# OrangeSodahub/InfGen

Hardware: AMD Instinct MI355X
Metric: agent-steps/sec (closed-loop rollout) (higher is better)
Workload: dtype f32

## Files before the change

### include/infgen_hip.h

```cpp
#ifndef INFGEN_HIP_H_
#define INFGEN_HIP_H_

#include <stdint.h>

#ifdef __cplusplus
extern "C" {
#endif

#define INFGEN_MAX_LAYERS 8

enum {
  INFGEN_Q_ATTN_PACK_SIZE = 0,
  INFGEN_Q_FOURIER_PACK_SIZE_N2 = 1,
  INFGEN_Q_FOURIER_PACK_SIZE_N3 = 2,
  INFGEN_Q_FOURIER_PACK_SIZE_N4 = 3,
  INFGEN_Q_TILE_ROWS = 4,
  INFGEN_Q_EDGE_ATTN_CAP = 5,
  INFGEN_Q_MAX_AGENTS = 6,
  INFGEN_Q_ABI_VERSION = 7,
  INFGEN_Q_SIZEOF_ROLLOUT = 8,
  INFGEN_Q_ATTN_SPLIT_ROWS = 9,
  INFGEN_Q_HEADS_SAMPLE_K = 10,
};
int infgen_layout_query(int what);
// ... 132 lines not shown
int infgen_heads(const float* X, int rows, const float* tok_pack, const float* st_pack, int token_size,
                 float* logits, int* next_token, int* next_state, void* stream);
int infgen_heads_logprob(const float* X, int rows, const float* tok_pack, const float* st_pack, int token_size,
                         float* logits, int* next_token, int* next_state, float* token_logprob, void* stream);
int infgen_token_logprob(const float* logits, int rows, int n, const int* token, float* out, void* stream);
int infgen_heads_sample(const float* X, int rows, const float* tok_pack, const float* st_pack, int token_size, int k,
                        const float* uniform, float* logits, int* next_token, int* next_state, float* token_logprob,
                        float* sample_logprob, void* stream);
int infgen_heads_sample_ex(const float* X, int rows, const float* tok_pack, const float* st_pack, int token_size, int k,
                           const float* uniform, const InfgenSampling* sampling, float* logits, int* next_token, int* next_state,
                           float* token_logprob, float* sample_logprob, void* stream);
int infgen_heads_sample_mask(const float* X, int rows, const float* tok_pack, const float* st_pack, int token_size, int k,
                             const float* uniform, const InfgenSampling* sampling, const uint32_t* mask_bits, int mask_n_sets,
                             const int* mask_row, const int* mask_type, const int* type, float* logits,
                             int* next_token, int* next_state, float* token_logprob, float* sample_logprob, void* stream);
int infgen_heads_sample_fused(int attn_mode, int rows, int k);
int infgen_heads_logprob_fused(int attn_mode, int rows);
int infgen_map_token_head(const float* X, int ldx, const int* gather, int n, const float* pack, int token_size,
                          float* hidden, float* logits, long long* top_idx, void* stream);
int infgen_embedding_sum4(const float* tab0, const long long* idx0, int n0, const float* tab1, const long long* idx1, int n1,
                          const float* tab2, const long long* idx2, int n2, const float* tab3, const long long* idx3, int n3,
                          int rows, float* out, void* stream);
int infgen_map_graph(int S, int M_cap, const int* n_map, const float* pos, const float* orient, float radius,
                     int max_nbr, int* off, int* cnt, int* src, float* raw, int* total, int cap, void* stream);

int infgen_rollout_validate(const InfgenRollout* r);
int infgen_build_edges(const InfgenRollout* r, int c, int edgeless, void* stream);
int infgen_integrate(const InfgenRollout* r, int t, void* stream);
int infgen_raw_feature(const InfgenRollout* r, int col, void* stream);
int infgen_raw_feature_rows(const InfgenRollout* r, int col, const int* row_list, const int* row_mask, int n, void* stream);
int infgen_decode_layers(const InfgenRollout* r, int c, int edgeless, void* stream);
int infgen_decode_step(const InfgenRollout* r, int t, void* stream);
int infgen_rollout_run(const InfgenRollout* r, int t0, int t1, void* stream);
int infgen_command_rows(const InfgenRollout* r, int t, int kind, const int* cmd_token, const float* cmd_pose,
                        const unsigned char* cmd_mask, const float* shape, float* cmd_cost, void* stream);

int infgen_branch_scenes(const InfgenRollout* r, int t, const int* parent, int* n_bad, void* stream);
int infgen_resample_parents(const int* ancestor, int S0, int copies, int* parent, void* stream);

int infgen_snapshot_bytes(const InfgenRollout* r, int t, long long* bytes);
int infgen_snapshot_scenes(const InfgenRollout* r, int t, const int* slots, int n, void* snap, long long entry_stride, int* head,
                           int* n_bad, void* stream);
int infgen_restore_scenes(const InfgenRollout* r, int t, const int* index, const void* snap, long long entry_stride, const int* head,
                          int n, int* n_bad, void* stream);

int infgen_sample_topk(const float* logits, int rows, int n, int k, const float* uniform, int* token, void* stream);
int infgen_sample_topk_logprob(const float* logits, int rows, int n, int k, const float* uniform, int* token,
                               float* sample_logprob, void* stream);
int infgen_sample_topk_ex(const float* logits, int rows, int n, int k, const float* uniform, const InfgenSampling* sampling,
                          int* token, float* sample_logprob, int* nucleus, void* stream);
int infgen_sample_topk_mask(const float* logits, int rows, int n, int k, const float* uniform, const InfgenSampling* sampling,
                            const uint32_t* mask_bits, int mask_n_sets, const int* mask_row, const int* mask_type, const int* type,
                            int* token, float* sample_logprob, int* nucleus, void* stream);
int infgen_token_mask_create(const uint32_t* mask_bits, int mask_n_sets, const int* mask_row, const int* mask_type, const int* type);
int infgen_token_mask_destroy(int handle);

int infgen_collision_end_poses(const float* vocab, int token_size, float* end_pose, void* stream);
int infgen_collision_mask(const float* pos, const float* head, const int* state, const int* n_agents, const int* first_new,
                          const int* type, const float* shape, int S, int A_cap, int T, int c, const float* end_pose, int token_size,
                          int predict, float margin, const uint32_t* mask_bits, int mask_n_sets, const int* mask_row,
                          const int* mask_type, uint32_t* out_bits, int* out_count, void* stream);
int infgen_token_mask_collision(int handle, uint32_t* dyn_bits, const int* identity_row, const float* shape, const float* end_pose,
                                int predict, float margin, int* count);

int infgen_road_records_from_map(const float* map_pos, const float* map_orient, const long long* map_type, const long long* map_tok,
                                 const int* n_map, int S0, int M_cap, const float* map_vocab, int n_token, int detail, float* records,
// ... 221 lines not shown
```

### infgen_amd/csrc/api.hip

```cpp
#include <cstdio>
#include <cstring>
#include <cstdlib>
#include <cmath>
#include <string>
#include <vector>
#include <atomic>
#include <mutex>
#include <unordered_map>
#include "kernels.h"
#include "../../include/infgen_hip.h"

using namespace ig;

static thread_local std::string g_err;

static int fail(const char* where, const char* what) {
  g_err = std::string(where) + ": " + what;
  return -1;
}
static int check_launch(const char* where) {
  hipError_t e = hipGetLastError();
  if (e != hipSuccess) return fail(where, hipGetErrorString(e));
  return 0;
}
// ... 81 lines not shown
static int env_layers_p() { const int v = env_int("INFGEN_LAYERS_P", 1); return v < 0 ? 0 : v > 2 ? 2 : v; }
static int env_lp_rows_min() {
  bool set8 = false;
  const int rows8 = env_int("INFGEN_LP_ROWS8", 0, &set8);
  return set8 ? (rows8 ? 8 : 16) : env_int("INFGEN_LP_ROWS_MIN", 4);
}
namespace knob {
const int layers_p = env_layers_p();
const int qs_dbg = env_int("INFGEN_QS_DBG", 0);
const int fh12_min = env_int("INFGEN_FH12_MIN", 150000);
const int fh12_multi_rows = env_int("INFGEN_FH12_MULTI_ROWS", 0);
const int fourier_nomulti = env_int("INFGEN_FOURIER_NOMULTI", 0);
const int attn_hs_max = env_int("INFGEN_ATTN_HS_MAX", 6144);
const int attn_waves = env_int("INFGEN_ATTN_WAVES", IG_QSU ? 8 : 4);
const int warm = env_int("INFGEN_WARM", 1);
const int warm_max_groups = env_int("INFGEN_WARM_MAX_GROUPS", 128);
const int edge_dbg = env_int("INFGEN_EDGE_DBG", 0);
const int edge_noxcd = env_int("INFGEN_EDGE_NOXCD", 0);
const int edge_small = env_int("INFGEN_EDGE_SMALL", 4096);
const int edge_wg2 = env_int("INFGEN_EDGE_WG2", 1);
const int edge_lds_pad = env_int("INFGEN_EDGE_LDS_PAD", 0);
const int heads_nosplit = env_int("INFGEN_HEADS_NOSPLIT", 0);
const int be_wide_scenes = env_int("INFGEN_BE_WIDE_SCENES", 128);
const int int_group_scenes = env_int("INFGEN_INT_GROUP_SCENES", 128);
const int no_tail_fold = env_int("INFGEN_NO_TAIL_FOLD", 0);
const int lp_max_chunks = env_int("INFGEN_LP_MAX_CHUNKS", 2);
const int lp_max_groups = env_int("INFGEN_LP_MAX_GROUPS", 256);
const int lp_rows_min = env_lp_rows_min();
const int cm_rows = env_int("INFGEN_CM_ROWS", 0);
const int lp_trace = env_int("INFGEN_LP_TRACE", 0);
const char* const lp_spin_str = getenv("INFGEN_LP_SPIN_LIMIT");
const unsigned lp_spin_limit = lp_spin_str ? (unsigned)strtoul(lp_spin_str, nullptr, 0) : 0u;
}

namespace {
InfgenOptions g_def = {0,  2,  3,  1,  1,  6,  0,
                        0,  knob::layers_p,  0,  1, 0, nullptr, nullptr};
int g_def_group_rows = 0;
const int* g_def_limit_n_agents = nullptr;
int g_def_limit_A_cap = 0;
struct Active { const InfgenOptions* o; int group_rows; const int* n_agents; int A_cap; };
thread_local Active tl_active = {nullptr, 0, nullptr, 0};
thread_local InfgenOptions tl_thread_opts;
thread_local bool tl_thread_set = false;
inline const InfgenOptions& O() { return tl_active.o ? *tl_active.o : tl_thread_set ? tl_thread_opts : g_def; }
inline int group_rows() { return tl_active.o ? tl_active.group_rows : g_def_group_rows; }
inline const int* limit_n_agents() { return tl_active.o ? tl_active.n_agents : g_def_limit_n_agents; }
inline int limit_A_cap() { return tl_active.o ? tl_active.A_cap : g_def_limit_A_cap; }
struct OptScope {
  Active prev;
  explicit OptScope(const InfgenRollout* r) : prev(tl_active) {
    if (r && r->opts.use) tl_active = Active{&r->opts, r->S * r->A_cap, r->opts.row_groups ? r->n_agents : nullptr, r->A_cap};
  }
  ~OptScope() { tl_active = prev; }
};
}

extern "C" int infgen_get_options(InfgenOptions* out) {
  if (!out) return fail("infgen_get_options", "null pointer");
  *out = g_def;
  return 0;
}

extern "C" int infgen_thread_options(const InfgenOptions* o) {
  if (o) { tl_thread_opts = *o; tl_thread_opts.row_groups = nullptr; tl_thread_opts.n_row_groups = nullptr; }
  tl_thread_set = o != nullptr;
  return 0;
}

extern "C" int infgen_get_effective_options(InfgenOptions* out) {
  if (!out) return fail("infgen_get_effective_options", "null pointer");
  *out = O();
  return 0;
}

namespace {
struct Prof {
  unsigned mask = 0;
  std::vector<hipEvent_t> e0, e1;
  std::vector<int> kid;
  std::vector<int> phase_of;
  std::vector<double> macs;
  int stride = 1;
  int seen[INFGEN_KID_COUNT] = {};
  int seen_step[INFGEN_KID_COUNT] = {};
  size_t used = 0;
  unsigned long long* rows_dev = nullptr;
} g_prof;

static thread_local int t_prof_phase = 0;
static std::mutex g_prof_mu;
struct ProfScope {
  int slot = -1;
  hipStream_t s;
  ProfScope(int kid, void* stream, double macs = 0.0) : s((hipStream_t)stream) {
    if ((g_prof.mask >> kid) & 1u) {
      std::lock_guard<std::mutex> lk(g_prof_mu);
      ++g_prof.seen[kid];
      const bool take = t_prof_phase != 1 || (g_prof.seen_step[kid]++ % g_prof.stride) == 0;
      if (take && g_prof.used < g_prof.e0.size()) {
        slot = (int)g_prof.used++;
        g_prof.kid[slot] = kid;
        g_prof.phase_of[slot] = t_prof_phase;
        g_prof.macs[slot] = macs;
        (void)hipEventRecord(g_prof.e0[slot], s);
      }
    }
// ... 201 lines not shown
extern "C" int infgen_set_gemm_terms(int terms) {
  if (terms < 1 || terms > 3) return fail("infgen_set_gemm_terms", "terms must be 3 (split, fp32 accuracy), 2 (bf16 operands) or 1 (fp16 operands)");
  g_def.gemm_terms = terms;
  return 0;
}

extern "C" int infgen_set_fourier_mode(int mode) {
  if (mode != 0 && mode != 1) return fail("infgen_set_fourier_mode", "mode must be 0 (fp32 MFMA) or 1 (fp16 split)");
  g_def.fourier_mode = mode;
  return 0;
}

static FourierArgs fourier_args(const float* raw, int n, const int* count_dev, int e_cap, const float* pack, const float* cat, int ldcat,
                                float* out, int ldo, int normalize, int out_r24, const float* dt_tab = nullptr, int dt_mode = 0) {
  return FourierArgs{raw, n, count_dev, e_cap, pack, cat, ldcat, out, ldo, normalize,
                     (g_prof.mask >> INFGEN_KID_FOURIER) & 1u && dt_mode != 2 ? g_prof.rows_dev : nullptr, out_r24, dt_tab, dt_mode, 0};
}

static inline int fourier_h_grid(int cap, bool wide) {
  const int grid = ceil_div(cap, wide ? FH12_TILE : FH_TILE);
  return grid > 256 * FH_WG_PER_CU ? 256 * FH_WG_PER_CU : grid;
}

static int launch_fourier(const FourierArgs& a_in, void* stream) {
  if (a_in.e_cap <= 0) return 0;
  FourierArgs a = a_in;
  a.dbg = knob::qs_dbg;
  { ProfScope _ps(INFGEN_KID_FOURIER, stream);
    if (O().fourier_mode == 0) {
      int grid = ceil_div(a.e_cap, TR);
      if (grid > 2048) grid = 2048;
      hipLaunchKernelGGL(k_fourier, dim3(grid), dim3(NT), 0, (hipStream_t)stream, a);
    } else {
      const bool wide = knob::fh12_min > 0 && a.e_cap >= knob::fh12_min && three_terms() && FH_WAVES == 8;
      const int grid = fourier_h_grid(a.e_cap, wide);
      if (wide) hipLaunchKernelGGL(k_fourier_h12<3>, dim3(grid), dim3(FH12_NT), 0, (hipStream_t)stream, a);
      else hipLaunchKernelGGL(by_terms(k_fourier_h<3>, k_fourier_h_b16<1>, k_fourier_h<1>), dim3(grid), dim3(FH_NT), 0, (hipStream_t)stream, a);
    } }
  return check_launch("infgen_fourier_embed");
}

static int fourier_embed_impl(const float* raw, int n, const int* count_dev, int e_cap, const float* pack,
                              const float* cat, int ldcat, float* out, int ldo, int normalize, int out_r24, void* stream,
                              const float* dt_tab = nullptr, int dt_mode = 0) {
  if (e_cap <= 0) return 0;
  if (n < 1 || n > 4) return fail("infgen_fourier_embed", "n_dims must be in 1..4");
  if (out_r24 && O().fourier_mode == 0) return fail("infgen_fourier_embed", "packed rows need the split kernel");
  if (dt_mode && (O().fourier_mode == 0 || n < 2 || (dt_mode == 1 && !dt_tab)))
    return fail("infgen_fourier_embed", "the last-dim table needs the split kernel, n_dims >= 2 and a table");
  return launch_fourier(fourier_args(raw, n, count_dev, e_cap, pack, cat, ldcat, out, ldo, normalize, out_r24, dt_tab, dt_mode), stream);
}

extern "C" int infgen_fourier_embed(const float* raw, int n, const int* count_dev, int e_cap, const float* pack,
                                    const float* cat, int ldcat, float* out, int ldo, int normalize, void* stream) {
  return fourier_embed_impl(raw, n, count_dev, e_cap, pack, cat, ldcat, out, ldo, normalize, 0, stream);
}

extern "C" int infgen_fourier_last_dim_table(const float* pack, int n, float* table, void* stream) {
  return fourier_embed_impl(nullptr, n, nullptr, DT_TAB_ROWS, pack, nullptr, 0, table, 128, 0, 0, stream, nullptr, 2);
}
extern "C" int infgen_fourier_embed_tab(const float* raw, int n, const int* count_dev, int e_cap, const float* pack,
                                        const float* table, float* out, int ldo, int normalize, void* stream) {
  return fourier_embed_impl(raw, n, count_dev, e_cap, pack, nullptr, 0, out, ldo, normalize, 0, stream, table, 1);
}

extern "C" int infgen_set_attn_mode(int mode) {
  if (mode < 0 || mode > 3) return fail("infgen_set_attn_mode", "mode must be 0 (fp32 MFMA), 1 (fp16 split), 2 (by size) or 3 (fp16 split, 16-row workgroups)");
// ... 1133 lines not shown
    if (coll.bits && (r->token_size % 32 || r->token_size > 64 * 32 * RIDER_WPL))
      return fail(where, "collision mask: token_size must be a multiple of 32, at most 4096");
    if (road.bits && (r->token_size % 32 || r->token_size > 64 * 32 * RIDER_WPL))
      return fail(where, "road mask: token_size must be a multiple of 32, at most 4096");
    if (road.bits && r->S % road.copies) return fail(where, "road mask: S must be a multiple of copies");
    if (score.out && r->first_new)
      return fail(where, "step score: contexts with scenario insertion cannot be scored: rows appended inside a step are left out");
    if (score.out && r->S % score.copies) return fail(where, "step score: S must be a multiple of copies");
  }
  if (r->token_logprob && !(r->store_logits && r->logits) && !r->logits_scratch) {
    const int mode = (r->opts.use ? r->opts : O()).attn_mode;
    const int k = r->sample_k > 1 && r->sample_u ? r->sample_k : 1;
    if (emit_plan(mode, r->S * r->A_cap, r->token_size, k, true, false).need_logits)
      return fail(where, "token_logprob needs store_logits or logits_scratch [rows][token_size] (few rows, or sampling)");
  }
  return 0;
}

static int build_edges_impl(const InfgenRollout* r, int c, int edgeless, void* stream, bool zero_totals, unsigned long long* clear_keys = nullptr,
                            bool clear_sync = false) {
  RET_IF(validate(r, "infgen_build_edges"));
  OptScope _opts(r);
  hipStream_t s = (hipStream_t)stream;
  if (!edgeless && zero_totals) {
    if (r->em.total == r->et.total + 1 && r->ea.total == r->et.total + 2) {
      if (hipMemsetAsync(r->et.total, 0, 3 * sizeof(int), s) != hipSuccess) return fail("infgen_build_edges", "memset failed");
    } else if (hipMemsetAsync(r->et.total, 0, sizeof(int), s) != hipSuccess ||
               hipMemsetAsync(r->em.total, 0, sizeof(int), s) != hipSuccess ||
               hipMemsetAsync(r->ea.total, 0, sizeof(int), s) != hipSuccess)
      return fail("infgen_build_edges", "memset failed");
  }
  BuildEdgesArgs a;
  a.st = scene_of(r); a.c = c; a.edgeless = edgeless; a.r_map = r->r_map; a.r_agent = r->r_agent;
  a.rows = r->S * r->A_cap; a.t = ebuf(r->et); a.m = ebuf(r->em); a.a = ebuf(r->ea);
  a.clear_keys = clear_keys;
  a.clear_sync = clear_sync ? reinterpret_cast<int*>(r->SIG) : nullptr;
  a.prof = (g_prof.mask & ((1u << INFGEN_KID_EDGE_ATTN) | (1u << INFGEN_KID_BUILD_EDGES))) ? g_prof.rows_dev : nullptr;
  { ProfScope _ps(INFGEN_KID_BUILD_EDGES, stream);
    a.map_lds = r->M_cap < 4096 ? r->M_cap : 4096;
    const size_t lds = (size_t)a.map_lds * 8;
    if (r->A_cap <= 256 && r->S > knob::be_wide_scenes) hipLaunchKernelGGL(k_build_edges<256>, dim3(r->S, 3), dim3(256), lds, s, a);
    else hipLaunchKernelGGL(k_build_edges<1024>, dim3(r->S, 3), dim3(1024), lds, s, a); }
  return check_launch("infgen_build_edges");
}
extern "C" int infgen_build_edges(const InfgenRollout* r, int c, int edgeless, void* stream) {
  return build_edges_impl(r, c, edgeless, stream, true);
}

static RawFeatArgs rawfeat_args(const InfgenRollout* r, int col) {
  RawFeatArgs a;
  a.st = scene_of(r); a.col = col; a.tok_tab = r->tok_tab; a.token_size = r->token_size;
  a.grid_tab = r->grid_tab; a.grid_size = r->grid_size; a.state_emb = r->state_emb;
  a.cat_agent = r->cat_agent; a.cat_seed = r->cat_seed; a.raw2 = r->raw2; a.cat = r->cat; a.fus_in = r->fus_in;
  a.row_list = nullptr; a.row_mask = nullptr; a.n_list = 0; a.no_grid = r->no_grid_token;
  return a;
}

static int integrate_groups(const InfgenRollout* r) {
  return (r->S <= knob::int_group_scenes && r->A_cap % 16 == 0 && r->A_cap > 16) ? r->A_cap / 16 : 1;
}
static int integrate_impl(const InfgenRollout* r, int t, void* stream, unsigned long long* heads_part, bool zero_totals, bool prep, bool zero_sync = false) {
  RET_IF(validate(r, "infgen_integrate"));
  OptScope _opts(r);
  IntegrateArgs a;
  a.heads_part = heads_part; a.next_token_w = r->next_token;
  a.edge_totals = zero_totals ? r->et.total : nullptr;
  a.zero_sync = zero_sync ? reinterpret_cast<int*>(r->SIG) : nullptr;
// ... 293 lines not shown
}
extern "C" int infgen_layers_p_capacity(void) {
  const LpDevice& d = lp_device();
  if (d.wg_per_cu <= 0) return 0;
  return d.n_cu * (d.wg_per_cu > 1 ? 1 : d.wg_per_cu);
}
static int lp_limit() {
  const int cap = infgen_layers_p_capacity(), mx = knob::lp_max_groups;
  return cap < mx ? cap : mx;
}
static bool is_capturing(void* stream) {
  hipStreamCaptureStatus cap = hipStreamCaptureStatusNone;
  return hipStreamIsCapturing((hipStream_t)stream, &cap) == hipSuccess && cap != hipStreamCaptureStatusNone;
}
static bool lp_packs_ok(const InfgenRollout* r, bool refresh = false, void* stream = nullptr) {
  static std::mutex mu;
  static std::unordered_map<const float*, bool> seen;
  std::lock_guard<std::mutex> lk(mu);
  const bool capturing = stream && is_capturing(stream);
  auto ok = [&](const float* pack) {
    if (!pack) return false;
    if (!refresh) { auto it = seen.find(pack); if (it != seen.end()) return it->second; }
    if (capturing) return false;
    float hdr[16] = {};
    const bool good = hipMemcpy(hdr, pack + AH_HDR, sizeof(hdr), hipMemcpyDeviceToHost) == hipSuccess && hdr[14] == AH_HDR_VERSION &&
                      hdr[10] > 0.f && hdr[12] > 0.f;
    seen[pack] = good;
    return good;
  };
  for (int i = 0; i < r->num_layers; ++i)
    if (!ok(r->attn_t[i]) || !ok(r->attn_m[i]) || !ok(r->attn_a[i])) return false;
  return true;
}
extern "C" int infgen_rollout_validate(const InfgenRollout* r) {
  RET_IF(validate(r, "infgen_rollout_validate"));
  if (r->replay_row && !(r->teacher_token && r->teacher_state))
    return fail("infgen_rollout_validate", "replay_row needs teacher_token and teacher_state (the plan the flagged rows follow)");
  if ((r->teacher_pos != nullptr) != (r->teacher_head != nullptr))
    return fail("infgen_rollout_validate", "teacher_pos and teacher_head come together");
  (void)lp_packs_ok(r, true);
  return 0;
}
static bool layers_p_shape(const InfgenRollout* r, int rows, int edgeless, void* stream) {
  const LpDevice& lpd = lp_device();
  if (lpd.wg_per_cu <= 0 || (O().layers_p == 2 && (!lpd.coop || g_lp_refused.load()))) return false;
  return O().layers_p && O().edge_fuse != 0 && O().attn_mode != 0 && three_terms() && O().fourier_mode != 0 &&
         !(O().overlap && g_side) && r->A_cap % 16 == 0 && lp_chunk_scenes(r, lp_limit()) > 0 &&
          r->num_layers <= LP_MAX_LAYERS && r->U && r->SIG && !r->tap_x && lp_packs_ok(r, false, stream);
}

struct StepMode { bool overlap, fuse, lp; int r24; int ra; const float* dt; };
static StepMode step_mode(const InfgenRollout* r, int rows, int edgeless, void* stream) {
  StepMode m;
  m.overlap = O().overlap && g_side && !edgeless;
  m.lp = layers_p_shape(r, rows, edgeless, stream);
  m.fuse = O().edge_fuse == 2 || (O().edge_fuse == 1 && (rows > 256 || m.lp));
  m.r24 = m.fuse && O().fourier_mode != 0 && O().rhat_format == 1;
  m.ra = m.r24;
  m.dt = O().fourier_mode != 0 ? r->four_t_dt : nullptr;
  return m;
}
static bool fourier_multi_ok(int rows, int edgeless) {
  return !edgeless && O().fourier_mode != 0 && rows <= 10240 && !knob::fourier_nomulti && !(O().overlap && g_side);
}

enum FourierSet { FS_TEMPORAL, FS_MAP, FS_AGENT, FS_XA };
static FourierArgs step_fourier_set(const InfgenRollout* r, FourierSet k, const StepMode& sm) {
  switch (k) {
    case FS_TEMPORAL:
      return fourier_args(r->et.raw, 4, r->et.total, r->et.cap, r->four_t, nullptr, 0, r->et.rhat, 128, 1, sm.r24, sm.dt, sm.dt != nullptr);
    case FS_MAP: return fourier_args(r->em.raw, 3, r->em.total, r->em.cap, r->four_m, nullptr, 0, r->em.rhat, 128, 1, sm.r24);
    case FS_AGENT: return fourier_args(r->ea.raw, 3, r->ea.total, r->ea.cap, r->four_a, nullptr, 0, r->ea.rhat, 128, 1, sm.ra);
    default: return fourier_args(r->raw2, 2, nullptr, r->S * r->A_cap, r->four_xa, r->cat, 128, r->fus_in + 128, 512, 0, 0);
// ... 13 lines not shown
    if (hipEventRecord(g_ev_m, g_side) != hipSuccess) return fail("infgen_decode_layers", "event failed");
    RET_IF(launch_fourier(step_fourier_set(r, FS_AGENT, sm), g_side));
    if (hipEventRecord(g_ev_a, g_side) != hipSuccess) return fail("infgen_decode_layers", "event failed");
    RET_IF(launch_fourier(step_fourier_set(r, FS_TEMPORAL, sm), stream));
  } else if (fourier_multi_ok(rows, edgeless)) {
    const int n_sets = with_xa ? 4 : 3;
    FourierMultiArgs m;
    for (int k = 0; k < n_sets; ++k) m.set[k] = step_fourier_set(r, (FourierSet)k, sm);
    int cap = r->et.cap > r->em.cap ? r->et.cap : r->em.cap;
    if (r->ea.cap > cap) cap = r->ea.cap;
    const bool wide = knob::fh12_multi_rows > 0 && rows >= knob::fh12_multi_rows && three_terms() && FH_WAVES == 8;
    const int grid = fourier_h_grid(cap, wide);
    { ProfScope _ps(INFGEN_KID_FOURIER, stream);
      if (wide) hipLaunchKernelGGL(k_fourier_h12_multi<3>, dim3(grid, n_sets), dim3(FH12_NT), 0, (hipStream_t)stream, m);
      else hipLaunchKernelGGL(by_terms(k_fourier_h_multi<3>, k_fourier_h_multi_b16<1>, k_fourier_h_multi<1>), dim3(grid, n_sets),
                              dim3(FH_NT), 0, (hipStream_t)stream, m); }
    RET_IF(check_launch("infgen_decode_layers(fourier)"));
  } else if (!edgeless) {
    for (FourierSet k : {FS_TEMPORAL, FS_MAP, FS_AGENT}) RET_IF(launch_fourier(step_fourier_set(r, k, sm), stream));
  }
  return 0;
}

constexpr int LP_REFUSED = -12345;
static int layers_p_launch(const InfgenRollout* r, int c, const StepMode& sm, void* stream, bool sync_clear = true) {
  const int rows = r->S * r->A_cap;
  LayersPArgs a;
  a.rows = rows; a.A_cap = r->A_cap; a.num_layers = r->num_layers;
  a.X = r->X;
  for (int i = 0; i < r->num_layers; ++i) {
    a.attn_t[i] = r->attn_t[i]; a.attn_m[i] = r->attn_m[i]; a.attn_a[i] = r->attn_a[i];
    a.ringK[i] = r->ringK[i]; a.ringV[i] = r->ringV[i]; a.mapK[i] = r->mapK[i]; a.mapV[i] = r->mapV[i];
  }
  a.slot_off = (size_t)(c % r->ring) * rows * D;
  a.Ka[0] = r->Ka; a.Va[0] = r->Va; a.Ka[1] = r->U; a.Va[1] = r->U + (size_t)rows * D;
  a.et = eset(r->et); a.em = eset(r->em); a.ea = eset(r->ea);
  a.sync = reinterpret_cast<int*>(r->SIG);
  a.trace = nullptr;
  const int lp_trace = knob::lp_trace;
  static unsigned long long* trace_dev = nullptr;
  if (lp_trace) {
    if (!trace_dev && hipMalloc(&trace_dev, 2048 * sizeof(unsigned long long)) != hipSuccess) return fail("infgen_decode_layers", "trace buffer");
    (void)hipMemsetAsync(trace_dev, 0, 2048 * sizeof(unsigned long long), (hipStream_t)stream);
    a.trace = trace_dev;
  }
  if (sync_clear && hipMemsetAsync(a.sync, 0, (size_t)r->S * sizeof(int), (hipStream_t)stream) != hipSuccess)
    return fail("infgen_decode_layers", "memset failed");
  const int limit = lp_limit();
  a.rows_per_wg = 16;
  for (int rr = 8; rr >= 4 && rr >= knob::lp_rows_min; rr >>= 1)
    if (r->A_cap % rr == 0 && rows / rr <= (rr == 4 ? limit / 2 : limit)) a.rows_per_wg = rr;
  const int gps = r->A_cap / a.rows_per_wg;
  const int per = rows / a.rows_per_wg <= limit ? r->S : (a.rows_per_wg == 16 ? lp_chunk_scenes(r, limit) : 0);
  if (per <= 0 || per * gps > infgen_layers_p_capacity()) return fail("infgen_decode_layers", "k_layers_p: batch does not fit the device's resident capacity");
  auto kern = a.rows_per_wg == 4 ? (sm.r24 ? k_layers_p<true, 4> : k_layers_p<false, 4>)
            : a.rows_per_wg == 8 ? (sm.r24 ? k_layers_p<true, 8> : k_layers_p<false, 8>)
                                 : (sm.r24 ? k_layers_p<true, 16> : k_layers_p<false, 16>);
  const bool capturing = is_capturing(stream);
  a.spin_limit = capturing ? (1u << 22) : knob::lp_spin_str ? knob::lp_spin_limit : (O().layers_p == 2 ? 0u : (1u << 24));
  std::unique_lock<std::mutex> lk(g_lp_mu, std::defer_lock);
  LpOrder& ord = g_lp_order[lp_current_device()];
  if (!capturing) {
    lk.lock();
    if (!ord.ev && hipEventCreateWithFlags(&ord.ev, hipEventDisableTiming) != hipSuccess)
      return fail("infgen_decode_layers", "event creation failed");
    if (ord.any && hipStreamWaitEvent((hipStream_t)stream, ord.ev, 0) != hipSuccess) {
      (void)hipGetLastError();
// ... 11 lines not shown
      hipLaunchKernelGGL(kern, dim3(n_wg), dim3(512), 0, (hipStream_t)stream, a);
    } else {
      void* params[] = {&a};
      const hipError_t e = hipLaunchCooperativeKernel(reinterpret_cast<const void*>(kern), dim3(n_wg), dim3(512), params, 0, (hipStream_t)stream);
      if (e != hipSuccess) {
        (void)hipGetLastError();
        if (s0 > 0) return fail("infgen_decode_layers", "k_layers_p: cooperative launch of a later chunk refused");
        g_lp_refused.store(true);
        return LP_REFUSED;
      }
    }
  }
  if (!capturing) {
    ord.any = hipEventRecord(ord.ev, (hipStream_t)stream) == hipSuccess;
    if (!ord.any) (void)hipGetLastError();
    lk.unlock();
  }
  if (lp_trace) {
    static int dumps = 0;
    if (dumps++ == lp_trace) {
      std::vector<unsigned long long> h(2048);
      (void)hipStreamSynchronize((hipStream_t)stream);
      (void)hipMemcpy(h.data(), trace_dev, 2048 * sizeof(unsigned long long), hipMemcpyDeviceToHost);
      for (int i = 0; i < 1024 && (i == 0 || h[2 * i + 1]); ++i)
        fprintf(stderr, "[lp trace] %d %llu %llu\n", i, h[2 * i], i ? h[2 * i + 1] - h[2 * i - 1] : 0ull);
    }
  }
  return check_launch("infgen_decode_layers(k_layers_p)");
}

static int layers_core(const InfgenRollout* r, int c, int edgeless, void* stream, bool lp_sync_clear = true) {
  const int rows = r->S * r->A_cap;
  const StepMode sm = step_mode(r, rows, edgeless, stream);
  if (sm.lp && sm.fuse) {
    const int rc = layers_p_launch(r, c, sm, stream, lp_sync_clear);
    if (rc != LP_REFUSED) return rc;
  }
  const bool overlap = sm.overlap, fuse = sm.fuse; const int r24 = sm.r24;
  const size_t slot = (size_t)(c % r->ring) * rows * D;
  const int L = r->num_layers;
  float* U = fuse ? nullptr : r->U;
  const float* Z = fuse ? nullptr : r->Z;
  const float* SIG = fuse ? nullptr : r->SIG;
  const int has_pos = fuse ? 0 : 1;
  const int QB = 16384;
  const bool skip_edges = edgeless && fuse;
  if (skip_edges && hipMemsetAsync(r->AGG, 0, (size_t)rows * D * sizeof(float), (hipStream_t)stream) != hipSuccess)
    return fail("infgen_decode_layers", "memset failed");
  auto edge = [&](const float* pack, const float* Ks, const float* Vs, const InfgenEdgeBuf& e, int kv_once = 0, const float* next_pack = nullptr, int fmt = -1) {
    if (skip_edges) return 0;
    if (fuse && O().attn_mode != 0)
      warm_request(pack + AH_POST + 4 * (QB / 4), 48 * QB, next_pack ? next_pack + AH_PRE : nullptr, 16 * QB);
    return fuse ? edge_fused_launch(rows, r->Q, pack, Ks, Vs, eset(e), r->AGG, r->A_cap, kv_once, stream, fmt < 0 ? r24 : fmt)
                : infgen_edge_attn(rows, r->Q, r->U, Ks, Vs, e.off, e.cnt, e.src, e.rhat, r->AGG, r->Z, r->SIG, stream);
  };
  RET_IF(infgen_attn_pre(r->X, rows, r->attn_t[0], 0, r->Q, U, r->ringK[0] + slot, r->ringV[0] + slot, stream));
  auto warm_post = [&](const float* pack) { if (fuse && O().attn_mode != 0) warm_request(pack + AH_POST, 52 * QB, nullptr, 0); };
  for (int i = 0; i < L; ++i) {
    RET_IF(edge(r->attn_t[i], r->ringK[i], r->ringV[i], r->et, 1, r->attn_m[i]));
    warm_post(r->attn_m[i]);
    RET_IF(infgen_attn_post_pre(r->X, rows, r->attn_t[i], r->AGG, Z, SIG, has_pos, r->attn_m[i], r->Q, U,
                                nullptr, nullptr, stream));
    if (overlap && i == 0 && hipStreamWaitEvent((hipStream_t)stream, g_ev_m, 0) != hipSuccess)
      return fail("infgen_decode_layers", "join failed");
    RET_IF(edge(r->attn_m[i], r->mapK[i], r->mapV[i], r->em, 0, r->attn_a[i]));
    warm_post(r->attn_a[i]);
    RET_IF(infgen_attn_post_pre(r->X, rows, r->attn_m[i], r->AGG, Z, SIG, has_pos, r->attn_a[i], r->Q, U,
                                r->Ka, r->Va, stream));
    if (overlap && i == 0 && hipStreamWaitEvent((hipStream_t)stream, g_ev_a, 0) != hipSuccess)
      return fail("infgen_decode_layers", "join failed");
    RET_IF(edge(r->attn_a[i], r->Ka, r->Va, r->ea, 0, i + 1 < L ? r->attn_t[i + 1] : nullptr, sm.ra));
    if (i + 1 < L) {
      warm_post(r->attn_t[i + 1]);
      RET_IF(infgen_attn_post_pre(r->X, rows, r->attn_a[i], r->AGG, Z, SIG, has_pos, r->attn_t[i + 1], r->Q, U,
                                  r->ringK[i + 1] + slot, r->ringV[i + 1] + slot, stream));
    } else {
      RET_IF(infgen_attn_post(r->X, rows, r->attn_a[i], r->AGG, Z, SIG, has_pos, stream));
    }
    if (r->tap_x && hipMemcpyAsync(r->tap_x + (size_t)i * rows * D, r->X, (size_t)rows * D * sizeof(float), hipMemcpyDeviceToDevice,
                                   (hipStream_t)stream) != hipSuccess)
      return fail("infgen_decode_layers", "tap copy failed");
  }
  return 0;
}

extern "C" int infgen_decode_layers(const InfgenRollout* r, int c, int edgeless, void* stream) {
  RET_IF(validate(r, "infgen_decode_layers"));
  OptScope _opts(r);
  ProfPhase _pp(edgeless ? t_prof_phase : 1);
  const StepMode sm = step_mode(r, r->S * r->A_cap, edgeless, stream);
  const bool lp = sm.lp && sm.fuse && r->SIG != nullptr;
  RET_IF(prepare_edges(r, c, edgeless, stream, true, false, nullptr, lp));
  return layers_core(r, c, edgeless, stream, !lp);
}

static EmitReq step_emit_req(const InfgenRollout* r, int t) {
  const int rows = r->S * r->A_cap;
  float* lg = (r->store_logits && r->logits) ? r->logits + (size_t)t * rows * r->token_size : nullptr;
  return EmitReq{r->X, rows, r->tok_head_pack, r->st_head_pack, r->token_size, lg, r->next_token, r->next_state};
}

extern "C" int infgen_decode_step(const InfgenRollout* r, int t, void* stream) {
  SamplingCtl ctl;
  StepRiders riders;
  RET_IF(validate(r, "infgen_decode_step", &ctl, &riders));
  auto& [mask, coll, road, score] = riders;
  OptScope _opts(r);
  ProfPhase _pp(1);
  const int rows = r->S * r->A_cap;
  const int c = 1 + t;
  if (t < 0 || c + 1 > r->T - 1) return fail("infgen_decode_step", "step beyond the column range");
  const RiderScene sc = rider_scene(r);
  RET_IF(infgen_decode_layers(r, c, 0, stream));
  if (coll.bits) {
    RET_IF(launch_collision("infgen_decode_step", collision_args(sc, c, coll, mask), stream));
    mask = TokenMaskCtl{coll.bits, rows, coll.ident, {-1, -1, -1}, nullptr};
  }
  if (road.bits) {
    RET_IF(launch_road("infgen_decode_step", road_args(sc, c, road, mask), stream));
    mask = TokenMaskCtl{road.bits, rows, road.ident, {-1, -1, -1}, nullptr};
  }
  EmitReq q = step_emit_req(r, t);
  q.ctl = ctl; q.mask = mask; q.mask_chain_heads = true;
  q.keys = reinterpret_cast<unsigned long long*>(r->tmp2);
  if (r->token_logprob) q.token_logprob = r->token_logprob + (size_t)t * rows;
  q.k = r->sample_u ? r->sample_k : 1;
  if (q.k > 1 && !q.logits && !r->logits_scratch && !emit_plan(q).sample_fused) q.k = 1;
  if (q.k > 1) {
    q.uniform = r->sample_u + (size_t)t * rows;
    if (r->sample_logprob) q.sample_logprob = r->sample_logprob + (size_t)t * rows;
  }
  const EmitPlan plan = emit_plan(q);
  if (plan.need_logits && !q.logits) q.logits = r->logits_scratch;
  RET_IF(emit_tokens("infgen_sample_topk", q, plan, stream));
  RET_IF(infgen_integrate(r, t, stream));
  if (score.out) {
    if (t >= score.steps) return fail("infgen_decode_step", "step score: the log holds fewer steps");
    RET_IF(launch_score("infgen_decode_step", score_args(sc, c + 1, score, score.out + (size_t)t * 8, (long long)score.steps * 8), stream));
  }
  RET_IF(infgen_raw_feature(r, c + 1, stream));
  return 0;
}

extern "C" int infgen_rollout_run(const InfgenRollout* r, int t0, int t1, void* stream) {
  StepRiders riders;
  RET_IF(validate(r, "infgen_rollout_run", nullptr, &riders));
  OptScope _opts(r);
  ProfPhase _pp(1);
  const int rows = r->S * r->A_cap;
  const bool sample = r->sample_k > 1 && r->sample_u;
  const bool fold = !knob::no_tail_fold && t1 > t0 && fourier_multi_ok(rows, 0) && O().attn_mode != 0 && !sample && !riders.any() && !r->token_logprob && !r->first_new &&
                    r->et.total && r->em.total == r->et.total + 1 && r->ea.total == r->et.total + 2;
  if (!fold) {
    for (int t = t0; t < t1; ++t) RET_IF(infgen_decode_step(r, t, stream));
    return 0;
  }
  if (t0 < 0 || 1 + t1 > r->T - 1) return fail("infgen_rollout_run", "step beyond the column range");
  unsigned long long* keys = reinterpret_cast<unsigned long long*>(r->tmp2);
  if (hipMemsetAsync(keys, 0, (size_t)rows * sizeof(unsigned long long), (hipStream_t)stream) != hipSuccess)
    return fail("infgen_rollout_run", "memset failed");
  const StepMode sm0 = step_mode(r, rows, 0, stream);
  const bool lp_steps = sm0.lp && sm0.fuse && r->SIG != nullptr;
  RET_IF(prepare_edges(r, 1 + t0, 0, stream, true, false, nullptr, lp_steps));
  for (int t = t0; t < t1; ++t) {
    const int c = 1 + t;
    RET_IF(layers_core(r, c, 0, stream, !lp_steps));
    EmitReq q = step_emit_req(r, t);
    q.keys = keys; q.keys_stay = true;
    bool split = false;
    RET_IF(emit_tokens("infgen_rollout_run", q, emit_plan(q), stream, &split));
    RET_IF(integrate_impl(r, t, stream, split ? keys : nullptr, t + 1 < t1, true, t + 1 < t1 && lp_steps));
    if (t + 1 < t1) {
      RET_IF(prepare_edges(r, c + 1, 0, stream, false, true, split && integrate_groups(r) > 1 ? keys : nullptr));
    } else {
      RET_IF(launch_fourier(step_fourier_set(r, FS_XA, sm0), stream));
    }
    RET_IF(raw_feature_fusion(r, stream));
  }
  return 0;
}

extern "C" int infgen_occupancy(const InfgenRollout* r, int c, float* occ, void* stream) {
  RET_IF(validate(r, "infgen_occupancy"));
  OccupancyArgs a{scene_of(r), c, r->grid_size, occ};
  hipLaunchKernelGGL(k_occupancy, dim3(r->S), dim3(NT), 0, (hipStream_t)stream, a);
  return check_launch("infgen_occupancy");
}

static int occupancy_embed_impl(const InfgenRollout* r, int c, float* occ, const float* embed_pack, float* emb, const int* active,
                                void* stream) {
  RET_IF(validate(r, "infgen_occupancy_embed"));
  if (r->grid_size > 2048) return fail("infgen_occupancy_embed", "grid larger than 2048 cells");
  OccEmbedArgs a{scene_of(r), c, r->grid_size, occ, embed_pack, emb, active};
  hipLaunchKernelGGL(k_occupancy_embed, dim3(r->S), dim3(NT), 0, (hipStream_t)stream, a);
  return check_launch("infgen_occupancy_embed");
}

extern "C" int infgen_occupancy_embed(const InfgenRollout* r, int c, float* occ, const float* embed_pack, float* emb, void* stream) {
  return occupancy_embed_impl(r, c, occ, embed_pack, emb, nullptr, stream);
}

extern "C" int infgen_point_edges(const InfgenRollout* r, int c, const int* centre_row, const int* active,
                                  int exclude_centre, int which, float r_agent, int k_agent, float r_map, int k_map,
                                  const InfgenEdgeBuf* ea, const InfgenEdgeBuf* em, void* stream) {
  RET_IF(validate(r, "infgen_point_edges"));
  hipStream_t s = (hipStream_t)stream;
  if (((which & 1) && hipMemsetAsync(ea->total, 0, sizeof(int), s) != hipSuccess) ||
      ((which & 2) && hipMemsetAsync(em->total, 0, sizeof(int), s) != hipSuccess))
    return fail("infgen_point_edges", "memset failed");
  PointEdgesArgs a{scene_of(r), c, centre_row, active, exclude_centre, which, r_agent, k_agent, r_map, k_map,
                   ebuf(*ea), ebuf(*em)};
// ... 301 lines not shown
```

Measured before the change: 29.62 million.

## Split rollout into two scene halves on parallel streams with phase offset

```diff
diff --git a/include/infgen_hip.h b/include/infgen_hip.h
--- a/include/infgen_hip.h
+++ b/include/infgen_hip.h
@@ -188,6 +188,7 @@
 int infgen_decode_layers(const InfgenRollout* r, int c, int edgeless, void* stream);
 int infgen_decode_step(const InfgenRollout* r, int t, void* stream);
 int infgen_rollout_run(const InfgenRollout* r, int t0, int t1, void* stream);
+int infgen_split_stats(int* split_runs, int* single_runs);
 int infgen_command_rows(const InfgenRollout* r, int t, int kind, const int* cmd_token, const float* cmd_pose,
                         const unsigned char* cmd_mask, const float* shape, float* cmd_cost, void* stream);
 
diff --git a/infgen_amd/csrc/api.hip b/infgen_amd/csrc/api.hip
--- a/infgen_amd/csrc/api.hip
+++ b/infgen_amd/csrc/api.hip
@@ -137,6 +137,8 @@
 const char* const lp_spin_str = getenv("INFGEN_LP_SPIN_LIMIT");
 const unsigned lp_spin_limit = lp_spin_str ? (unsigned)strtoul(lp_spin_str, nullptr, 0) : 0u;
 }
+static int split_halves_knob() { return env_int("INFGEN_SPLIT_HALVES", 1); }
+static int split_offset_knob() { return env_int("INFGEN_SPLIT_OFFSET", 4); }
 
 namespace {
 InfgenOptions g_def = {0,  2,  3,  1,  1,  6,  0,
@@ -178,6 +180,10 @@
   *out = O();
   return 0;
 }
+
+struct SplitTl { int full_rows; int cap_scale; hipEvent_t mark_ev; int mark_at; };
+static thread_local SplitTl tl_split = {0, 1, nullptr, -1};
+static inline int stride_rows(const InfgenRollout* r) { return tl_split.full_rows ? tl_split.full_rows : r->S * r->A_cap; }
 
 namespace {
 struct Prof {
@@ -445,7 +451,7 @@
       if (grid > 2048) grid = 2048;
       hipLaunchKernelGGL(k_fourier, dim3(grid), dim3(NT), 0, (hipStream_t)stream, a);
     } else {
-      const bool wide = knob::fh12_min > 0 && a.e_cap >= knob::fh12_min && three_terms() && FH_WAVES == 8;
+      const bool wide = knob::fh12_min > 0 && (long long)a.e_cap * tl_split.cap_scale >= knob::fh12_min && three_terms() && FH_WAVES == 8;
       const int grid = fourier_h_grid(a.e_cap, wide);
       if (wide) hipLaunchKernelGGL(k_fourier_h12<3>, dim3(grid), dim3(FH12_NT), 0, (hipStream_t)stream, a);
       else hipLaunchKernelGGL(by_terms(k_fourier_h<3>, k_fourier_h_b16<1>, k_fourier_h<1>), dim3(grid), dim3(FH_NT), 0, (hipStream_t)stream, a);
@@ -1645,7 +1651,7 @@
   }
   BuildEdgesArgs a;
   a.st = scene_of(r); a.c = c; a.edgeless = edgeless; a.r_map = r->r_map; a.r_agent = r->r_agent;
-  a.rows = r->S * r->A_cap; a.t = ebuf(r->et); a.m = ebuf(r->em); a.a = ebuf(r->ea);
+  a.rows = stride_rows(r); a.t = ebuf(r->et); a.m = ebuf(r->em); a.a = ebuf(r->ea);
   a.clear_keys = clear_keys;
   a.clear_sync = clear_sync ? reinterpret_cast<int*>(r->SIG) : nullptr;
   a.prof = (g_prof.mask & ((1u << INFGEN_KID_EDGE_ATTN) | (1u << INFGEN_KID_BUILD_EDGES))) ? g_prof.rows_dev : nullptr;
@@ -2005,6 +2011,7 @@
     if (!ok(r->attn_t[i]) || !ok(r->attn_m[i]) || !ok(r->attn_a[i])) return false;
   return true;
 }
+static bool split_copy_boundary(const InfgenRollout* r, bool refresh);
 extern "C" int infgen_rollout_validate(const InfgenRollout* r) {
   RET_IF(validate(r, "infgen_rollout_validate"));
   if (r->replay_row && !(r->teacher_token && r->teacher_state))
@@ -2012,6 +2019,7 @@
   if ((r->teacher_pos != nullptr) != (r->teacher_head != nullptr))
     return fail("infgen_rollout_validate", "teacher_pos and teacher_head come together");
   (void)lp_packs_ok(r, true);
+  (void)split_copy_boundary(r, true);
   return 0;
 }
 static bool layers_p_shape(const InfgenRollout* r, int rows, int edgeless, void* stream) {
@@ -2091,7 +2099,7 @@
     a.attn_t[i] = r->attn_t[i]; a.attn_m[i] = r->attn_m[i]; a.attn_a[i] = r->attn_a[i];
     a.ringK[i] = r->ringK[i]; a.ringV[i] = r->ringV[i]; a.mapK[i] = r->mapK[i]; a.mapV[i] = r->mapV[i];
   }
-  a.slot_off = (size_t)(c % r->ring) * rows * D;
+  a.slot_off = (size_t)(c % r->ring) * stride_rows(r) * D;
   a.Ka[0] = r->Ka; a.Va[0] = r->Va; a.Ka[1] = r->U; a.Va[1] = r->U + (size_t)rows * D;
   a.et = eset(r->et); a.em = eset(r->em); a.ea = eset(r->ea);
   a.sync = reinterpret_cast<int*>(r->SIG);
@@ -2169,12 +2177,18 @@
 static int layers_core(const InfgenRollout* r, int c, int edgeless, void* stream, bool lp_sync_clear = true) {
   const int rows = r->S * r->A_cap;
   const StepMode sm = step_mode(r, rows, edgeless, stream);
+  bool marked = tl_split.mark_ev == nullptr;
+  auto mark = [&](int sublayer, bool last) {
+    if (marked || !(last || sublayer >= tl_split.mark_at)) return 0;
+    marked = true;
+    return hipEventRecord(tl_split.mark_ev, (hipStream_t)stream) == hipSuccess ? 0 : fail("infgen_rollout_run", "phase mark failed");
+  };
   if (sm.lp && sm.fuse) {
     const int rc = layers_p_launch(r, c, sm, stream, lp_sync_clear);
-    if (rc != LP_REFUSED) return rc;
+    if (rc != LP_REFUSED) { if (rc == 0) RET_IF(mark(0, true)); return rc; }
   }
   const bool overlap = sm.overlap, fuse = sm.fuse; const int r24 = sm.r24;
-  const size_t slot = (size_t)(c % r->ring) * rows * D;
+  const size_t slot = (size_t)(c % r->ring) * stride_rows(r) * D;
   const int L = r->num_layers;
   float* U = fuse ? nullptr : r->U;
   const float* Z = fuse ? nullptr : r->Z;
@@ -2198,12 +2212,14 @@
     warm_post(r->attn_m[i]);
     RET_IF(infgen_attn_post_pre(r->X, rows, r->attn_t[i], r->AGG, Z, SIG, has_pos, r->attn_m[i], r->Q, U,
                                 nullptr, nullptr, stream));
+    RET_IF(mark(3 * i, false));
     if (overlap && i == 0 && hipStreamWaitEvent((hipStream_t)stream, g_ev_m, 0) != hipSuccess)
       return fail("infgen_decode_layers", "join failed");
     RET_IF(edge(r->attn_m[i], r->mapK[i], r->mapV[i], r->em, 0, r->attn_a[i]));
     warm_post(r->attn_a[i]);
     RET_IF(infgen_attn_post_pre(r->X, rows, r->attn_m[i], r->AGG, Z, SIG, has_pos, r->attn_a[i], r->Q, U,
                                 r->Ka, r->Va, stream));
+    RET_IF(mark(3 * i + 1, false));
     if (overlap && i == 0 && hipStreamWaitEvent((hipStream_t)stream, g_ev_a, 0) != hipSuccess)
       return fail("infgen_decode_layers", "join failed");
     RET_IF(edge(r->attn_a[i], r->Ka, r->Va, r->ea, 0, i + 1 < L ? r->attn_t[i + 1] : nullptr, sm.ra));
@@ -2214,6 +2230,7 @@
     } else {
       RET_IF(infgen_attn_post(r->X, rows, r->attn_a[i], r->AGG, Z, SIG, has_pos, stream));
     }
+    RET_IF(mark(3 * i + 2, i + 1 == L));
     if (r->tap_x && hipMemcpyAsync(r->tap_x + (size_t)i * rows * D, r->X, (size_t)rows * D * sizeof(float), hipMemcpyDeviceToDevice,
                                    (hipStream_t)stream) != hipSuccess)
       return fail("infgen_decode_layers", "tap copy failed");
@@ -2233,7 +2250,7 @@
 
 static EmitReq step_emit_req(const InfgenRollout* r, int t) {
   const int rows = r->S * r->A_cap;
-  float* lg = (r->store_logits && r->logits) ? r->logits + (size_t)t * rows * r->token_size : nullptr;
+  float* lg = (r->store_logits && r->logits) ? r->logits + (size_t)t * stride_rows(r) * r->token_size : nullptr;
   return EmitReq{r->X, rows, r->tok_head_pack, r->st_head_pack, r->token_size, lg, r->next_token, r->next_state};
 }
 
@@ -2260,12 +2277,12 @@
   EmitReq q = step_emit_req(r, t);
   q.ctl = ctl; q.mask = mask; q.mask_chain_heads = true;
   q.keys = reinterpret_cast<unsigned long long*>(r->tmp2);
-  if (r->token_logprob) q.token_logprob = r->token_logprob + (size_t)t * rows;
+  if (r->token_logprob) q.token_logprob = r->token_logprob + (size_t)t * stride_rows(r);
   q.k = r->sample_u ? r->sample_k : 1;
   if (q.k > 1 && !q.logits && !r->logits_scratch && !emit_plan(q).sample_fused) q.k = 1;
   if (q.k > 1) {
-    q.uniform = r->sample_u + (size_t)t * rows;
-    if (r->sample_logprob) q.sample_logprob = r->sample_logprob + (size_t)t * rows;
+    q.uniform = r->sample_u + (size_t)t * stride_rows(r);
+    if (r->sample_logprob) q.sample_logprob = r->sample_logprob + (size_t)t * stride_rows(r);
   }
   const EmitPlan plan = emit_plan(q);
   if (plan.need_logits && !q.logits) q.logits = r->logits_scratch;
@@ -2279,41 +2296,196 @@
   return 0;
 }
 
-extern "C" int infgen_rollout_run(const InfgenRollout* r, int t0, int t1, void* stream) {
+struct RunPlan { bool fold = false, lp_steps = false; unsigned long long* keys = nullptr; StepMode sm0{}; };
+static int run_begin(const InfgenRollout* r, int t0, int t1, void* stream, RunPlan* p) {
   StepRiders riders;
   RET_IF(validate(r, "infgen_rollout_run", nullptr, &riders));
   OptScope _opts(r);
   ProfPhase _pp(1);
   const int rows = r->S * r->A_cap;
   const bool sample = r->sample_k > 1 && r->sample_u;
-  const bool fold = !knob::no_tail_fold && t1 > t0 && fourier_multi_ok(rows, 0) && O().attn_mode != 0 && !sample && !riders.any() && !r->token_logprob && !r->first_new &&
-                    r->et.total && r->em.total == r->et.total + 1 && r->ea.total == r->et.total + 2;
-  if (!fold) {
-    for (int t = t0; t < t1; ++t) RET_IF(infgen_decode_step(r, t, stream));
+  p->fold = !knob::no_tail_fold && t1 > t0 && fourier_multi_ok(rows, 0) && O().attn_mode != 0 && !sample && !riders.any() && !r->token_logprob && !r->first_new &&
+            r->et.total && r->em.total == r->et.total + 1 && r->ea.total == r->et.total + 2;
+  if (!p->fold) return 0;
+  if (t0 < 0 || 1 + t1 > r->T - 1) return fail("infgen_rollout_run", "step beyond the column range");
+  p->keys = reinterpret_cast<unsigned long long*>(r->tmp2);
+  if (hipMemsetAsync(p->keys, 0, (size_t)rows * sizeof(unsigned long long), (hipStream_t)stream) != hipSuccess)
+    return fail("infgen_rollout_run", "memset failed");
+  p->sm0 = step_mode(r, rows, 0, stream);
+  p->lp_steps = p->sm0.lp && p->sm0.fuse && r->SIG != nullptr;
+  return prepare_edges(r, 1 + t0, 0, stream, true, false, nullptr, p->lp_steps);
+}
+static int run_step(const InfgenRollout* r, int t, int t1, void* stream, const RunPlan& p) {
+  if (!p.fold) return infgen_decode_step(r, t, stream);
+  OptScope _opts(r);
+  ProfPhase _pp(1);
+  const int c = 1 + t;
+  RET_IF(layers_core(r, c, 0, stream, !p.lp_steps));
+  EmitReq q = step_emit_req(r, t);
+  q.keys = p.keys; q.keys_stay = true;
+  bool split = false;
+  RET_IF(emit_tokens("infgen_rollout_run", q, emit_plan(q), stream, &split));
+  RET_IF(integrate_impl(r, t, stream, split ? p.keys : nullptr, t + 1 < t1, true, t + 1 < t1 && p.lp_steps));
+  if (t + 1 < t1) {
+    RET_IF(prepare_edges(r, c + 1, 0, stream, false, true, split && integrate_groups(r) > 1 ? p.keys : nullptr));
+  } else {
+    RET_IF(launch_fourier(step_fourier_set(r, FS_XA, p.sm0), stream));
+  }
+  return raw_feature_fusion(r, stream);
+}
+
+namespace {
+struct SplitRes {
+  hipStream_t st[2] = {nullptr, nullptr};
+  hipEvent_t fork = nullptr, join[2] = {nullptr, nullptr}, mark = nullptr;
+  int* totals = nullptr;
+};
+std::mutex g_split_mu;
+std::unordered_map<void*, SplitRes> g_split_res;
+constexpr size_t SPLIT_MAX_STREAMS = 8;
+std::atomic<int> g_split_runs{0}, g_single_runs{0};
+std::mutex g_split_copy_mu;
+std::unordered_map<const int*, std::pair<int, bool>> g_split_copy_ok;
+}
+extern "C" int infgen_split_stats(int* split_runs, int* single_runs) {
+  if (split_runs) *split_runs = g_split_runs.load();
+  if (single_runs) *single_runs = g_single_runs.load();
+  return 0;
+}
+static SplitRes* split_res(void* stream) {
+  auto it = g_split_res.find(stream);
+  if (it != g_split_res.end()) return &it->second;
+  if (g_split_res.size() >= SPLIT_MAX_STREAMS) return nullptr;
+  SplitRes v;
+  bool ok = hipMalloc(&v.totals, 8 * sizeof(int)) == hipSuccess;
+  for (int h = 0; h < 2 && ok; ++h)
+    ok = hipStreamCreateWithFlags(&v.st[h], hipStreamNonBlocking) == hipSuccess &&
+         hipEventCreateWithFlags(&v.join[h], hipEventDisableTiming) == hipSuccess;
+  ok = ok && hipEventCreateWithFlags(&v.fork, hipEventDisableTiming) == hipSuccess &&
+       hipEventCreateWithFlags(&v.mark, hipEventDisableTiming) == hipSuccess;
+  if (!ok) { (void)hipGetLastError(); return nullptr; }
+  return &(g_split_res[stream] = v);
+}
+static bool split_copy_boundary(const InfgenRollout* r, bool refresh) {
+  if (!r->map_scene || r->S < 2 || r->S % 2) return true;
+  std::lock_guard<std::mutex> lk(g_split_copy_mu);
+  auto it = g_split_copy_ok.find(r->map_scene);
+  if (!refresh && it != g_split_copy_ok.end() && it->second.first == r->S) return it->second.second;
+  int mid[2] = {0, 0};
+  const bool ok = hipMemcpy(mid, r->map_scene + r->S / 2 - 1, sizeof(mid), hipMemcpyDeviceToHost) == hipSuccess && mid[0] != mid[1];
+  (void)hipGetLastError();
+  g_split_copy_ok[r->map_scene] = {r->S, ok};
+  return ok;
+}
+static bool run_split_mode(const InfgenRollout* r, int t0, int t1, void* stream) {
+  const int mode = split_halves_knob();
+  if (mode <= 0 || t1 <= t0 || r->S < 2 || r->S % 2) return false;
+  if (r->first_new || O().row_groups || r->token_mask || r->tap_x || g_prof.mask || tl_split.full_rows) return false;
+  if (r->et.cap < 2 || r->em.cap < 2 || r->ea.cap < 2 || !r->et.total || !r->em.total || !r->ea.total) return false;
+  if (is_capturing(stream)) return false;
+  if (mode == 1) {
+    const int rows = r->S * r->A_cap, half = r->S / 2;
+    if (rows / 2 <= 10240 || rows / 2 <= knob::edge_small || rows / 2 <= knob::attn_hs_max) return false;
+    if ((r->S > knob::be_wide_scenes) != (half > knob::be_wide_scenes) || (r->S > knob::int_group_scenes) != (half > knob::int_group_scenes)) return false;
+    if (step_mode(r, rows, 0, stream).lp) return false;
+  }
+  return split_copy_boundary(r, false);
+}
+static InfgenRollout split_half(const InfgenRollout* r, int h, int* totals) {
+  InfgenRollout q = *r;
+  q.S = r->S / 2;
+  const size_t s0 = h ? (size_t)q.S : 0, A = r->A_cap, row0 = s0 * A, col0 = s0 * r->T * A, m0 = s0 * r->M_cap;
+  auto adv = [](auto*& p, size_t n) { if (p) p += n; };
+  adv(q.n_agents, s0); adv(q.av_index, s0);
+  if (q.map_scene) adv(q.map_scene, s0);
+  else { adv(q.n_map, s0); adv(q.map_pos, 2 * m0); adv(q.map_orient, m0); }
+  adv(q.pos, 2 * col0); adv(q.head, col0); adv(q.state, col0); adv(q.token, col0); adv(q.grid, col0);
+  adv(q.tmask, col0); adv(q.imask, col0); adv(q.catflag, col0); adv(q.type, row0); adv(q.bos, row0);
+  adv(q.cat_agent, row0 * D);
+  for (int l = 0; l < INFGEN_MAX_LAYERS; ++l) {
+    adv(q.ringK[l], row0 * D); adv(q.ringV[l], row0 * D);
+    if (!q.map_scene) { adv(q.mapK[l], m0 * D); adv(q.mapV[l], m0 * D); }
+  }
+  adv(q.X, row0 * D); adv(q.Q, row0 * D); adv(q.U, row0 * 8 * D); adv(q.Ka, row0 * D); adv(q.Va, row0 * D); adv(q.AGG, row0 * D);
+  adv(q.Z, row0 * 8 * D); adv(q.SIG, row0 * 8);
+  int k = 0;
+  for (InfgenEdgeBuf* e : {&q.et, &q.em, &q.ea}) {
+    const int capA = e->cap / 2;
+    adv(e->off, row0); adv(e->cnt, row0);
+    if (h) { adv(e->src, (size_t)capA); adv(e->raw, (size_t)capA * 4); adv(e->rhat, (size_t)capA * D); }
+    e->cap = h ? e->cap - capA : capA;
+    e->total = totals + 3 * h + k++;
+  }
+  adv(q.raw2, row0 * 4); adv(q.cat, row0 * D); adv(q.fus_in, row0 * 512); adv(q.tmp1, row0 * D); adv(q.tmp2, row0 * D);
+  adv(q.next_token, row0); adv(q.next_state, row0); adv(q.logits, row0 * r->token_size);
+  adv(q.teacher_token, col0); adv(q.teacher_state, col0); adv(q.teacher_grid, col0); adv(q.teacher_pos, 2 * col0); adv(q.teacher_head, col0);
+  adv(q.replay_row, row0);
+  adv(q.pred_traj, row0 * r->R * 2); adv(q.pred_head, row0 * r->R); adv(q.pred_state, row0 * r->R);
+  adv(q.sample_u, row0); adv(q.logits_scratch, row0 * r->token_size); adv(q.sample_temp_row, row0);
+  adv(q.sample_logprob, row0); adv(q.token_logprob, row0);
+  q.opts = O(); q.opts.use = 1;
+  q.opts.overlap = 0;
+  return q;
+}
+__global__ void k_split_totals(const int* half, int* t, int* m, int* a, int cap_t, int cap_m, int cap_a) {
+  if (threadIdx.x >= 3 || blockIdx.x) return;
+  const int k = threadIdx.x, cap = k == 0 ? cap_t : k == 1 ? cap_m : cap_a, capA = cap / 2;
+  const int na = half[k], nb = half[3 + k];
+  int n = na + nb;
+  if ((na > capA || nb > cap - capA) && n <= cap) n = cap + 1;
+  *(k == 0 ? t : k == 1 ? m : a) = n;
+}
+static int run_split(const InfgenRollout* r, int t0, int t1, void* stream, SplitRes& res) {
+  hipStream_t cs = (hipStream_t)stream;
+  const int full_rows = r->S * r->A_cap;
+  InfgenRollout half[2] = {split_half(r, 0, res.totals), split_half(r, 1, res.totals)};
+  const int L3 = 3 * r->num_layers;
+  const int off_knob = split_offset_knob(), off = off_knob < 0 ? 0 : off_knob > L3 ? L3 : off_knob;
+  if (hipEventRecord(res.fork, cs) != hipSuccess || hipStreamWaitEvent(res.st[0], res.fork, 0) != hipSuccess ||
+      hipStreamWaitEvent(res.st[1], res.fork, 0) != hipSuccess)
+    return fail("infgen_rollout_run", "fork failed");
+  struct TlScope { ~TlScope() { tl_split = SplitTl{0, 1, nullptr, -1}; } } _tl;
+  auto body = [&]() {
+    RunPlan plan[2];
+    for (int h = 0; h < 2; ++h) {
+      tl_split = SplitTl{full_rows, 2, nullptr, -1};
+      RET_IF(run_begin(&half[h], t0, t1, res.st[h], &plan[h]));
+    }
+    for (int t = t0; t < t1; ++t) {
+      tl_split = SplitTl{full_rows, 2, off > 0 ? res.mark : nullptr, off - 1};
+      RET_IF(run_step(&half[0], t, t1, res.st[0], plan[0]));
+      tl_split = SplitTl{full_rows, 2, nullptr, -1};
+      if (off > 0 && hipStreamWaitEvent(res.st[1], res.mark, 0) != hipSuccess) return fail("infgen_rollout_run", "phase wait failed");
+      RET_IF(run_step(&half[1], t, t1, res.st[1], plan[1]));
+    }
     return 0;
-  }
-  if (t0 < 0 || 1 + t1 > r->T - 1) return fail("infgen_rollout_run", "step beyond the column range");
-  unsigned long long* keys = reinterpret_cast<unsigned long long*>(r->tmp2);
-  if (hipMemsetAsync(keys, 0, (size_t)rows * sizeof(unsigned long long), (hipStream_t)stream) != hipSuccess)
-    return fail("infgen_rollout_run", "memset failed");
-  const StepMode sm0 = step_mode(r, rows, 0, stream);
-  const bool lp_steps = sm0.lp && sm0.fuse && r->SIG != nullptr;
-  RET_IF(prepare_edges(r, 1 + t0, 0, stream, true, false, nullptr, lp_steps));
-  for (int t = t0; t < t1; ++t) {
-    const int c = 1 + t;
-    RET_IF(layers_core(r, c, 0, stream, !lp_steps));
-    EmitReq q = step_emit_req(r, t);
-    q.keys = keys; q.keys_stay = true;
-    bool split = false;
-    RET_IF(emit_tokens("infgen_rollout_run", q, emit_plan(q), stream, &split));
-    RET_IF(integrate_impl(r, t, stream, split ? keys : nullptr, t + 1 < t1, true, t + 1 < t1 && lp_steps));
-    if (t + 1 < t1) {
-      RET_IF(prepare_edges(r, c + 1, 0, stream, false, true, split && integrate_groups(r) > 1 ? keys : nullptr));
-    } else {
-      RET_IF(launch_fourier(step_fourier_set(r, FS_XA, sm0), stream));
+  };
+  const int rc = body();
+  bool joined = true;
+  for (int h = 0; h < 2; ++h)
+    joined = hipEventRecord(res.join[h], res.st[h]) == hipSuccess && hipStreamWaitEvent(cs, res.join[h], 0) == hipSuccess && joined;
+  if (rc) return rc;
+  if (!joined) return fail("infgen_rollout_run", "join failed");
+  hipLaunchKernelGGL(k_split_totals, dim3(1), dim3(64), 0, cs, res.totals, r->et.total, r->em.total, r->ea.total, r->et.cap, r->em.cap, r->ea.cap);
+  return check_launch("infgen_rollout_run(totals)");
+}
+
+extern "C" int infgen_rollout_run(const InfgenRollout* r, int t0, int t1, void* stream) {
+  RET_IF(validate(r, "infgen_rollout_run"));
+  {
+    OptScope _opts(r);
+    if (run_split_mode(r, t0, t1, stream)) {
+      std::lock_guard<std::mutex> lk(g_split_mu);
+      if (SplitRes* res = split_res(stream)) {
+        ++g_split_runs;
+        return run_split(r, t0, t1, stream, *res);
+      }
     }
-    RET_IF(raw_feature_fusion(r, stream));
-  }
+  }
+  ++g_single_runs;
+  RunPlan plan;
+  RET_IF(run_begin(r, t0, t1, stream, &plan));
+  for (int t = t0; t < t1; ++t) RET_IF(run_step(r, t, t1, stream, plan));
   return 0;
 }
 
```

New measurement: 30.37 million (median of 6 runs). 2.5% higher.
